# cipherflow-fhe/lattisense

Measured on AMD Instinct MI355X. Metric: ckks_hmult_relin_rescale_throughput, higher is better.
Workload: dtype u64

## Files before the change

lattisense_amd/csrc/build_flags.h:

```cpp
#pragma once

#if (defined(LSA_NTT_DIAG_NO_TWIDDLE_LOADS) || defined(LSA_NTT_DIAG_COPY_ONLY) || defined(LSA_NTT_DIAG_COMPUTE_ONLY) || defined(LSA_NTT_DIAG_TW8) || \
     defined(LSA_KS_DIAG_NO_MATH) || defined(LSA_KS_DIAG_NO_STORE) || defined(LSA_BC_DIAG_NO_MATH) || defined(LSA_BC_DIAG_NO_STORE)) && \
    !defined(LSA_DIAG_BUILD)
#error "wrong-result diagnostic switches need -DLSA_DIAG_BUILD (use lattisense_amd.build --variant: it adds the flag and renames the library)"
#endif

#define LSA_BF_STR2(x) #x
#define LSA_BF_STR(x) LSA_BF_STR2(x)

#define LSA_BUILD_FLAGS_TEXT_1 ""
#ifdef LSA_DIAG_BUILD
#define LSA_BF_DIAG " LSA_DIAG_BUILD"
#else
#define LSA_BF_DIAG ""
#endif
#ifdef LSA_NTT_DIAG_NO_TWIDDLE_LOADS
#define LSA_BF_A " LSA_NTT_DIAG_NO_TWIDDLE_LOADS"
#else
#define LSA_BF_A ""
#endif
#ifdef LSA_NTT_DIAG_COPY_ONLY
#define LSA_BF_B " LSA_NTT_DIAG_COPY_ONLY"
#else
// ... 89 lines not shown
#else
#define LSA_BF_T ""
#endif
#if defined(LSA_NTT_HEAD_ROUNDS) && LSA_NTT_HEAD_ROUNDS != 2
#define LSA_BF_U " LSA_NTT_HEAD_ROUNDS=" LSA_BF_STR(LSA_NTT_HEAD_ROUNDS)
#else
#define LSA_BF_U ""
#endif
#ifdef LSA_R16_BARRIERS
#define LSA_BF_X " LSA_R16_BARRIERS"
#else
#define LSA_BF_X ""
#endif
#if defined(LSA_R16_WAVES) && LSA_R16_WAVES != 4
#define LSA_BF_Y " LSA_R16_WAVES=" LSA_BF_STR(LSA_R16_WAVES)
#else
#define LSA_BF_Y ""
#endif
#ifdef LSA_NTT_NO_LAZY
#define LSA_BF_Z " LSA_NTT_NO_LAZY"
#else
#define LSA_BF_Z ""
#endif
#ifdef LSA_SHOUP_SINGLE_ASM
#define LSA_BF_AA " LSA_SHOUP_SINGLE_ASM"
#else
#define LSA_BF_AA ""
#endif
#ifdef LSA_AB_DPP_LO
#define LSA_BF_AB " LSA_AB_DPP_LO"
#else
#define LSA_BF_AB ""
#endif
#if defined(LSA_KSMAC_WAVES) && LSA_KSMAC_WAVES != 2
#define LSA_BF_AC " LSA_KSMAC_WAVES=" LSA_BF_STR(LSA_KSMAC_WAVES)
#else
#define LSA_BF_AC ""
#endif
#if defined(LSA_KSMAC_WAVES_FP) && LSA_KSMAC_WAVES_FP != 2
#define LSA_BF_AE " LSA_KSMAC_WAVES_FP=" LSA_BF_STR(LSA_KSMAC_WAVES_FP)
#else
#define LSA_BF_AE ""
#endif
#if defined(LSA_KSMAC_CHUNK) && LSA_KSMAC_CHUNK != 4
#define LSA_BF_AF " LSA_KSMAC_CHUNK=" LSA_BF_STR(LSA_KSMAC_CHUNK)
#else
#define LSA_BF_AF ""
#endif
#if defined(LSA_KSMAC_TWCACHE) && LSA_KSMAC_TWCACHE != 1
#define LSA_BF_AH " LSA_KSMAC_TWCACHE=" LSA_BF_STR(LSA_KSMAC_TWCACHE)
#else
#define LSA_BF_AH ""
#endif
#ifdef LSA_NTT_DIAG_TW8
#define LSA_BF_AD " LSA_NTT_DIAG_TW8"
#else
#define LSA_BF_AD ""
#endif
#ifdef LSA_LIFT_ROW_OUTER
#define LSA_BF_AG " LSA_LIFT_ROW_OUTER"
#else
#define LSA_BF_AG ""
#endif
#ifdef LSA_VARIANT_NAME
#define LSA_BF_V " variant=" LSA_BF_STR(LSA_VARIANT_NAME)
#else
#define LSA_BF_V ""
#endif
#ifdef LSA_AB_SWITCH
#define LSA_BF_W " LSA_AB_SWITCH=" LSA_BF_STR(LSA_AB_SWITCH)
#else
#define LSA_BF_W ""
#endif

#define LSA_BUILD_FLAGS_TEXT                                                                                              \
    LSA_BF_DIAG LSA_BF_A LSA_BF_B LSA_BF_C LSA_BF_D LSA_BF_E LSA_BF_F LSA_BF_G LSA_BF_H LSA_BF_I LSA_BF_J LSA_BF_K LSA_BF_L \
        LSA_BF_M LSA_BF_N LSA_BF_O LSA_BF_P LSA_BF_Q LSA_BF_R LSA_BF_S LSA_BF_T LSA_BF_U LSA_BF_V LSA_BF_W LSA_BF_X LSA_BF_Y LSA_BF_Z LSA_BF_AA LSA_BF_AB LSA_BF_AC LSA_BF_AD LSA_BF_AE LSA_BF_AF LSA_BF_AG LSA_BF_AH
```

lattisense_amd/csrc/emu_ntt.cpp:

```cpp
#define LSA_EMULATE 1
#include <cstddef>
#include <vector>
#include "ntt_plan.h"
#include "ntt_chunk.h"
#include "ntt_r16.h"
#include <array>
#include "tables.h"

template <int NT>
static void emu_block(const NttPassArgs& a, const NttBlockCtx& bc, u64* lds) {
    for (int t = 0; t < NT; t++) ntt_phase_load<true, NT, true>(a, bc, t, lds);
    int rho[4];
    const int np = ntt_split(a.mu, rho);
    if (!a.inverse) {
        int sig = 0;
        for (int i = 0; i < np; i++) {
            for (int t = 0; t < NT; t++) ntt_phase_sub_dyn<NT>(a, bc, t, lds, sig, rho[i]);
            sig += rho[i];
        }
    } else {
        int sig = a.mu;
        for (int i = np - 1; i >= 0; i--) {
            sig -= rho[i];
            for (int t = 0; t < NT; t++) ntt_phase_sub_dyn<NT>(a, bc, t, lds, sig, rho[i]);
        }
    }
    for (int t = 0; t < NT; t++) ntt_phase_store<true, NT>(a, bc, t, lds);
}

template <int PASS, int MU, int FZ = 3 | 16>
static void emu_block_r16(const NttPassArgs& a, const NttBlockCtx& bc, u64* lds) {
    std::vector<std::array<u64, 16>> regs(LSA_R16_THREADS);
    for (int phase = 0; phase < 3; phase++)
        for (int t = 0; t < LSA_R16_THREADS; t++) {
            u64(&v)[16] = *reinterpret_cast<u64(*)[16]>(regs[t].data());
            r16_phase<PASS, FZ, MU>(a, bc, t, lds, phase, v);
        }
}

static void emu_block_r8x3(const NttPassArgs& a, const NttBlockCtx& bc, u64* lds) {
    std::vector<std::array<u64, 16>> regs(LSA_R16_THREADS);
    for (int phase = 0; phase < 4; phase++)
        for (int t = 0; t < LSA_R16_THREADS; t++) {
            u64(&v)[16] = *reinterpret_cast<u64(*)[16]>(regs[t].data());
            r8x3_phase<3 | 16>(a, bc, t, lds, phase, v);
        }
}

static int emu_ntt(int n, const u64* moduli, int nmod, u64* data, int batch, long long batch_stride, int rows,
                   const unsigned char* mod_of, int period, int inverse, int tau_max, int allow_fp64, const u64* pa, const u64* pb,
                   const u64* lift = nullptr, int lift_mod = 0, int lift_limbs = 1, int chunk = 0, long long sa = -1,
                   long long sb = -1, long long slift = -1) {
    const int row_inner = (allow_fp64 >> 1) & 1;
    const bool r16 = (allow_fp64 >> 2) & 1;
    allow_fp64 &= 1;
    lsa::HostTables T;
    T.build(n, std::vector<u64>(moduli, moduli + nmod));
    NttPlan plan = make_ntt_plan(T.logn, tau_max);
    std::vector<u64> tw_i(T.psi.size());
    std::vector<double> tw_d(T.psi_d.size());
    for (int m = 0; m < nmod; m++) {
        const size_t o = (size_t)m * n;
        ntt_permute_twiddles(plan, T.logn, (inverse ? T.psiinv : T.psi).data() + 2 * o, tw_i.data() + 2 * o, 2, false);
        ntt_permute_twiddles(plan, T.logn, (inverse ? T.psiinv_d : T.psi_d).data() + o, tw_d.data() + o, 1, true);
    }
    NttPassArgs a{};
    a.src = data;
    a.dst = data;
    a.src_stride = batch_stride;
    a.dst_stride = batch_stride;
    a.batch = batch;
    a.rows = rows;
    a.mods = T.mods.data();
    a.tw = tw_i.data();
    a.scale = T.scale.data();
    a.twd = tw_d.data();
    a.scaled = T.scale_d.data();
    a.allow_fp64 = allow_fp64;
    a.period = period;
    a.row0 = 0;
    a.row_step = 1;
    a.row_inner = row_inner;
    for (int i = 0; i < period; i++) a.mod_of[i] = mod_of[i];
    if (pa) {
        a.fz_pro = 3;
        a.fz_limbs = rows;
        a.fz_a = pa;
        a.fz_b = pb;
        a.fz_a_stride = sa >= 0 ? sa : batch_stride;
        a.fz_b_stride = sb >= 0 ? sb : batch_stride;
        a.fz_a_rpp = a.fz_b_rpp = rows;
    }
    if (lift) {
        a.fz_pro = 4;
        a.fz_limbs = lift_limbs;
        a.fz_last = lift;
        a.fz_last_stride = slift >= 0 ? slift : (long long)(rows / lift_limbs) * n;
        a.fz_last_rpp = 1;
        a.fz_ql_mod = lift_mod;
    }
    int launch_rows = 0;
    for (int r = 0; r < rows; r++)
        if (mod_of[r % period] != LSA_ROW_SKIP) a.row_tbl[launch_rows++] = (unsigned short)r;
    a.compact = 1;
    a.rows = launch_rows;
    const NttPassArgs whole = a;
    const int items = chunk > 0 && chunk < batch ? chunk : batch;
    for (int b0 = 0; b0 < batch; b0 += items) {
        const int nb = batch - b0 < items ? batch - b0 : items;
        a = ntt_chunk_rebase(whole, b0);
        a.batch = nb;
        a.src = a.dst = data + (long long)b0 * batch_stride;
        for (int step = 0; step < plan.npass; step++) {
            int k = inverse ? plan.npass - 1 - step : step;
            ntt_fill_pass(a, plan, T.logn, k, inverse);
            a.fz_first = step == 0;
            a.fp_raw_out = plan.npass == 2 && step == 0;
            a.fp_raw_in = plan.npass == 2 && step == 1;
            std::vector<u64> lds(lds_words(a.tau));
            long long nblocks = (long long)nb * launch_rows * (1 << (a.logn - a.tau));
            for (long long bid = 0; bid < nblocks; bid++) {
                NttBlockCtx bc = ntt_decode_block(a, bid);
                if (bc.mod == LSA_ROW_SKIP) continue;
                if (r16 && ntt_r16_shape_ok(a, plan.npass)) {
                    if (a.mu == 9) emu_block_r8x3(a, bc, lds.data());
                    else if (a.lambda && lift) (a.mu == 8 ? emu_block_r16<0, 8, 32> : emu_block_r16<0, 7, 32>)(a, bc, lds.data());
                    else if (a.lambda && a.mu == 8) emu_block_r16<0, 8>(a, bc, lds.data());
                    else if (a.lambda) emu_block_r16<0, 7>(a, bc, lds.data());
                    else if (a.mu == 8) emu_block_r16<1, 8>(a, bc, lds.data());
                    else emu_block_r16<1, 7>(a, bc, lds.data());
                } else if (a.tau <= 12) emu_block<LSA_NTT_THREADS>(a, bc, lds.data());
                else if (a.tau == 13) emu_block<512>(a, bc, lds.data());
                else emu_block<1024>(a, bc, lds.data());
            }
        }
    }
    return 0;
}

extern "C" int lsa_emu_ntt(int n, const u64* moduli, int nmod, u64* data, int batch, long long batch_stride, int rows,
                           const unsigned char* mod_of, int period, int inverse, int tau_max, int allow_fp64) {
    return emu_ntt(n, moduli, nmod, data, batch, batch_stride, rows, mod_of, period, inverse, tau_max, allow_fp64, nullptr, nullptr);
}

extern "C" int lsa_emu_intt_prod(int n, const u64* moduli, int nmod, const u64* pa, const u64* pb, u64* out, int batch,
                                 long long batch_stride, int rows, const unsigned char* mod_of, int period, int tau_max,
                                 int allow_fp64) {
    if (!pa || !pb) return -1;
    return emu_ntt(n, moduli, nmod, out, batch, batch_stride, rows, mod_of, period, 1, tau_max, allow_fp64, pa, pb);
}

extern "C" int lsa_emu_ntt_lift(int n, const u64* moduli, int nmod, const u64* src, int src_mod, int limbs, u64* out, int batch,
                                long long batch_stride, int rows, const unsigned char* mod_of, int period, int tau_max,
                                int allow_fp64) {
    if (!src || limbs < 1 || rows % limbs || src_mod < 0 || src_mod + rows / limbs > nmod) return -1;
    return emu_ntt(n, moduli, nmod, out, batch, batch_stride, rows, mod_of, period, 0, tau_max, allow_fp64, nullptr, nullptr, src,
                   src_mod, limbs);
}

extern "C" int lsa_emu_intt_prod_chunked(int n, const u64* moduli, int nmod, const u64* pa, long long sa, const u64* pb, long long sb,
                                         u64* out, int batch, long long batch_stride, int rows, const unsigned char* mod_of,
                                         int period, int tau_max, int allow_fp64, int chunk) {
    if (!pa || !pb || sa < 0 || sb < 0 || chunk < 0) return -1;
    return emu_ntt(n, moduli, nmod, out, batch, batch_stride, rows, mod_of, period, 1, tau_max, allow_fp64, pa, pb, nullptr, 0, 1,
                   chunk, sa, sb);
}

extern "C" int lsa_emu_ntt_lift_chunked(int n, const u64* moduli, int nmod, const u64* src, long long src_stride, int src_mod,
                                        int limbs, u64* out, int batch, long long batch_stride, int rows,
                                        const unsigned char* mod_of, int period, int tau_max, int allow_fp64, int chunk) {
    if (!src || src_stride < 0 || limbs < 1 || rows % limbs || src_mod < 0 || src_mod + rows / limbs > nmod || chunk < 0) return -1;
    return emu_ntt(n, moduli, nmod, out, batch, batch_stride, rows, mod_of, period, 0, tau_max, allow_fp64, nullptr, nullptr, src,
// ... 3 lines not shown
```

lattisense_amd/csrc/kernels.hip:

```cpp
#include <atomic>
#include <cstdlib>

#include "build_flags.h"
#include "ks_mac_groups.h"
#include "lsa_internal.h"
#include "ntt_r16.h"
#include "plain_ops.h"
#include "poly_lincomb.h"
#include "tensor_sum.h"

namespace lsa {

const char* kernels_build_flags() { return LSA_BUILD_FLAGS_TEXT; }

static constexpr int TPB = 256;

#ifndef LSA_NTT_WAVES
#define LSA_NTT_WAVES 4
#endif

#if defined(LSA_NTT_DIAG_STAMPS)
#define LSA_STAMP(k)                                                                               \
    do {                                                                                           \
        if (a.diag && threadIdx.x == 0 && blockIdx.x < 8192) a.diag[blockIdx.x * 8 + (k)] = __builtin_amdgcn_s_memtime(); \
// ... 54 lines not shown
    __syncthreads();
    ntt_butterfly_phases<NT>(a, bc, tid, lds);
    if (lds[lds_addr(tid)] == 0x123456789abcull) a.dst[bc.base_dst + tid] = 1;
    return;
#endif
    LSA_STAMP(0);
    ntt_phase_load<(FZ & 1) != 0, NT, (FZ & 16) != 0>(a, bc, tid, lds);
    if (TWL && tid < (1 << a.mu)) {
        u64* tw_l = lds + lds_words(a.tau);
        if (bc.fp) tw_l[tid] = twp.x;
        else {
            tw_l[2 * tid] = twp.x;
            tw_l[2 * tid + 1] = twp.y;
        }
    }
    LSA_STAMP(1);
    __syncthreads();
    LSA_STAMP(2);
#if defined(LSA_NTT_DIAG_COPY_ONLY)
    ntt_phase_store<(FZ & 2) != 0, NT, (FZ & 4) != 0, (FZ & 8) != 0>(a, bc, tid, lds);
    return;
#endif
    ntt_butterfly_phases<NT, TWL>(a, bc, tid, lds);
    ntt_phase_store<(FZ & 2) != 0, NT, (FZ & 4) != 0, (FZ & 8) != 0>(a, bc, tid, lds);
    LSA_STAMP(7);
}

template <int PASS>
__device__ __forceinline__ void r16_sync() {
#if defined(LSA_R16_BARRIERS)
    __syncthreads();
#else
    if (PASS == 0) {
        __syncthreads();
    } else {
        __builtin_amdgcn_fence(__ATOMIC_RELEASE, "wavefront");
        __builtin_amdgcn_wave_barrier();
        __builtin_amdgcn_fence(__ATOMIC_ACQUIRE, "wavefront");
    }
#endif
}
#ifndef LSA_R16_WAVES
#define LSA_R16_WAVES 4
#endif
template <int PASS, int FZ, int MU>
__global__ __launch_bounds__(LSA_R16_THREADS, (FZ & 1) ? LSA_NTT_WAVES_FUSED : LSA_R16_WAVES) void k_ntt_r16(NttPassArgs a) {
    extern __shared__ __attribute__((aligned(16))) u64 lds[];
    const int tid = threadIdx.x;
    const NttBlockCtx bc = ntt_decode_block(a, (long long)blockIdx.x);
    if (bc.mod == LSA_ROW_SKIP) return;
    u64 v[16];
    r16_phase<PASS, FZ, MU>(a, bc, tid, lds, 0, v);
    if (!(PASS == 0 && a.inverse)) r16_sync<PASS>();
    r16_phase<PASS, FZ, MU>(a, bc, tid, lds, 1, v);
    if (PASS == 0 && !a.inverse) return;
    r16_sync<PASS>();
    r16_phase<PASS, FZ, MU>(a, bc, tid, lds, 2, v);
}
template <int FZ>
__global__ __launch_bounds__(LSA_R16_THREADS, LSA_R16_WAVES) void k_ntt_r8x3(NttPassArgs a) {
    extern __shared__ __attribute__((aligned(16))) u64 lds[];
    const int tid = threadIdx.x;
    const NttBlockCtx bc = ntt_decode_block(a, (long long)blockIdx.x);
    if (bc.mod == LSA_ROW_SKIP) return;
    u64 v[16];
    r8x3_phase<FZ>(a, bc, tid, lds, 0, v);
    r16_sync<1>();
    r8x3_phase<FZ>(a, bc, tid, lds, 1, v);
    r16_sync<1>();
    r8x3_phase<FZ>(a, bc, tid, lds, 2, v);
    r16_sync<1>();
    r8x3_phase<FZ>(a, bc, tid, lds, 3, v);
}
static int ntt_pass_fz(const NttPassArgs& a, bool fused) {
    const bool pro = fused && a.fz_pro && a.fz_first, epi = fused && a.fz_epi && a.final_reduce;
    if (pro && a.fz_pro == 3) return 16;
    if (epi && a.fz_epi == 3) return 4;
    if (epi && a.fz_epi == 4) return 8;
    return (pro ? 1 : 0) | (epi ? 2 : 0);
}
template <int FZ>
static auto ntt_r16_second_pass(int mu) {
    return mu == 9 ? &k_ntt_r8x3<FZ> : mu == 8 ? &k_ntt_r16<1, FZ, 8> : &k_ntt_r16<1, FZ, 7>;
}
static bool ntt_launch_r16(const NttPassArgs& a, int npass, bool fused, long long nblocks, hipStream_t s) {
    if (!sw::ntt_r16() || !ntt_r16_shape_ok(a, npass)) return false;
    const int fz = ntt_pass_fz(a, fused);
    void (*k)(NttPassArgs) = nullptr;
    if (a.lambda) {
        if (fz == 1 && a.fz_pro == 4 && sw::r16_pro()) k = a.mu == 8 ? &k_ntt_r16<0, 32, 8> : &k_ntt_r16<0, 32, 7>;
        else if (fz == 1 && a.fz_pro != 4 && a.mu == 8 && sw::r16_pro()) k = &k_ntt_r16<0, 1, 8>;
        else if (fz == 0) k = a.mu == 8 ? &k_ntt_r16<0, 0, 8> : &k_ntt_r16<0, 0, 7>;
    } else if (a.mu != 9 || sw::ntt_r8x3()) {
        switch (fz) {
            case 0: k = ntt_r16_second_pass<0>(a.mu); break;
            case 2: k = ntt_r16_second_pass<2>(a.mu); break;
            case 4: k = ntt_r16_second_pass<4>(a.mu); break;
            case 8: k = ntt_r16_second_pass<8>(a.mu); break;
            case 16: k = a.inverse ? ntt_r16_second_pass<16>(a.mu) : nullptr; break;
        }
    }
    if (!k) return false;
    hipLaunchKernelGGL(k, dim3((unsigned)nblocks), dim3(LSA_R16_THREADS), (size_t)LSA_R16_LDS_WORDS * sizeof(u64), s, a);
    LSA_HIP(hipGetLastError());
    return true;
}

#ifndef LSA_KSMAC_WAVES
#define LSA_KSMAC_WAVES 2
#endif
#ifndef LSA_KSMAC_WAVES_FP
#define LSA_KSMAC_WAVES_FP LSA_KSMAC_WAVES
#endif
template <int MU, bool FP, bool TAIL = false>
__global__ __launch_bounds__(LSA_R16_THREADS, FP ? LSA_KSMAC_WAVES_FP : LSA_KSMAC_WAVES) void k_ntt_r16_ksmac(KsFusedArgs g) {
    static_assert(!TAIL || (FP && MU <= 8), "the tail runs on the FP64 engine's eight- and seven-stage passes");
    extern __shared__ __attribute__((aligned(16))) u64 lds[];
    const int tid = threadIdx.x;
    const int T = g.L + g.np;
    long long bid = blockIdx.x;
    long long b;
    if (g.xcd_deal) {
        const long long slot = bid >> 3;
        b = slot % g.batch;
        bid = (slot / g.batch) * 8 + (bid & 7);
    } else {
        b = bid % g.batch;
        bid /= g.batch;
    }
    const int tl = g.tl_list[bid % g.n_tl], tile = (int)(bid / g.n_tl);
    NttPassArgs a;
    a.logn = g.logn;
    a.s_lo = g.logn - MU;
    a.mu = MU;
    a.lambda = 0;
    a.tau = 12;
    a.inverse = 0;
    a.apply_scale = 0;
    a.final_reduce = 1;
    a.fp_raw_in = g.fp_raw_in;
    a.fp_raw_out = 0;
    a.mods = g.mods;
    a.tw = g.tw;
    a.twd = g.twd;
    a.scale = nullptr;
    a.scaled = nullptr;
    a.src = g.ext;
    a.fz_pro = a.fz_epi = 0;
    a.fz_first = 0;
    NttBlockCtx bc;
    bc.tile = tile;
    bc.mod = tl < g.L ? tl : g.nq + (tl - g.L);
    bc.fp = FP;
    bc.b = (int)b;
    bc.row = 0;
    bc.tw_l = nullptr;
// ... 2379 lines not shown
```

lattisense_amd/csrc/ntt_core.h:

```cpp
#pragma once
#include "modarith.h"

#ifndef LSA_NTT_THREADS
#define LSA_NTT_THREADS 256
#endif
#define LSA_MAX_PERIOD 192
#if defined(LSA_EMULATE)
#include <cstdio>
#include <cstdlib>
#define LSA_EMU_CHECK(c) do { if (!(c)) { std::fprintf(stderr, "ntt replay: range invariant violated: %s (%s:%d)\n", #c, __FILE__, __LINE__); std::abort(); } } while (0)
#else
#define LSA_EMU_CHECK(c) do { } while (0)
#endif
#define LSA_ROW_SKIP 0xFF
#define LSA_FP64_MAX_BITS 47
#ifndef LSA_NTT_MAX_RHO
#define LSA_NTT_MAX_RHO 4
#endif

struct NttPassArgs {
    const u64* src;
    u64* dst;
    long long src_stride;
    long long dst_stride;
// ... 698 lines not shown
    const u64* pa;
    const u64* pb;
    const int half = 1 << (a.tau - 1);
    const NttStoreFix f = ntt_make_store_fix<FZ>(a, bc, g, pa, pb);
    const NttTileMap tm = ntt_tile_map(a, bc.tile);
    if (half == LSA_NTT_STAGE_PAIRS * NT) {
        for (int p0 = 0; p0 < LSA_NTT_STAGE_PAIRS; p0 += LSA_NTT_STORE_CHUNK) {
            u64 v[2 * LSA_NTT_STORE_CHUNK], va[2 * LSA_NTT_STORE_CHUNK], vb[2 * LSA_NTT_STORE_CHUNK];
            int xs[LSA_NTT_STORE_CHUNK];
#pragma unroll
            for (int p = 0; p < LSA_NTT_STORE_CHUNK; p++) {
                const int l = 2 * (tid + (p0 + p) * NT);
                const int x = ntt_tile_index(tm, l);
                xs[p] = x;
                v[2 * p] = lds[lds_addr(l)];
                v[2 * p + 1] = lds[lds_addr(l + 1)];
                va[2 * p] = va[2 * p + 1] = vb[2 * p] = vb[2 * p + 1] = 0;
                if (f.tail) {
                    ntt_load_data_pair(pa + x, va[2 * p], va[2 * p + 1]);
                }
                if (f.with_base) {
                    ntt_load_data_pair(pb + x, vb[2 * p], vb[2 * p + 1]);
                }
            }
            if (FZ && f.tail && a.fz_scatter) {
#pragma unroll
                for (int p = 0; p < LSA_NTT_STORE_CHUNK; p++) {
                    g[a.fz_scatter[xs[p]]] = ntt_store_fix(f, v[2 * p], va[2 * p], vb[2 * p]);
                    g[a.fz_scatter[xs[p] + 1]] = ntt_store_fix(f, v[2 * p + 1], va[2 * p + 1], vb[2 * p + 1]);
                }
                continue;
            }
#pragma unroll
            for (int p = 0; p < LSA_NTT_STORE_CHUNK; p++)
                ntt_store_pair(g + xs[p], ntt_store_fix(f, v[2 * p], va[2 * p], vb[2 * p]),
                               ntt_store_fix(f, v[2 * p + 1], va[2 * p + 1], vb[2 * p + 1]));
        }
        return;
    }
    for (int i = tid; i < half; i += NT) {
        const int x = ntt_tile_index(tm, 2 * i);
        const u64 a0 = f.tail ? pa[x] : 0, a1 = f.tail ? pa[x + 1] : 0;
        const u64 b0 = f.with_base ? pb[x] : 0, b1 = f.with_base ? pb[x + 1] : 0;
        const u64 w0 = ntt_store_fix(f, lds[lds_addr(2 * i)], a0, b0), w1 = ntt_store_fix(f, lds[lds_addr(2 * i + 1)], a1, b1);
        if (FZ && f.tail && a.fz_scatter) {
            g[a.fz_scatter[x]] = w0;
            g[a.fz_scatter[x + 1]] = w1;
        } else {
            ntt_store_pair(g + x, w0, w1);
        }
    }
}

template <int RHO, bool TWU, bool lazy>
LSA_HD void ntt_group_int_impl(u64 (&v)[1 << RHO], bool inverse, const u64* tw , int s_base, unsigned G, u64 q_,
                               bool scale_here, u64 sc0, u64 sc0s, u64 sc1, u64 sc1s) {
    constexpr int E = 1 << RHO;
    const u64 q = q_;
#if defined(LSA_NTT_EXACT_BFLY)
    const u64 q2 = 2 * q;
#else
    const u64 q4 = 4 * q, nq = 0 - q, nq4 = 0 - q4;
#endif
    if (!inverse) {
#pragma unroll
        for (int j = 0; j < RHO; j++) {
            const int half = E >> (j + 1);
            const int s = s_base + j;
            const u64* tws = tw + 2 * (1LL << s);
            u64 w[E / 2], ws[E / 2];
#if defined(LSA_NTT_DIAG_TW8)
            if (!TWU) {
                double wd[E / 2];
                ntt_load_tw_fp(reinterpret_cast<const double*>(tw) + (1LL << s), s, j, G, wd);
#pragma unroll
                for (int k = 0; k < (1 << j); k++) {
                    w[k] = (u64)__builtin_bit_cast(long long, wd[k]);
                    ws[k] = (w[k] << 3) | 1;
                }
            } else
#endif
#pragma unroll
            for (int k = 0; k < (1 << j); k++) {
                if (TWU) {
                    w[k] = LSA_CONST_PTR(u64, tws)[2 * ntt_tw_u_int(s, j, k) + 2u * ntt_tw_v_int(j, G)];
                    ws[k] = LSA_CONST_PTR(u64, tws)[2 * ntt_tw_u_int(s, j, k) + 2u * ntt_tw_v_int(j, G) + 1];
                } else {
                    ntt_load_pair(tws + 2 * ntt_tw_u_int(s, j, k) + 2u * ntt_tw_v_int(j, G), w[k], ws[k]);
                }
            }
#pragma unroll
            for (int e = 0; e < E; e++) {
                if ((e & half) == 0) {
                    const int k = e >> (RHO - j);
#if defined(LSA_NTT_DIAG_NO_TWIDDLE_LOADS)
                    const u64 wk = (u64)(G + 2 * k + 3), wsk = (u64)(G + 2 * k + 5) << 40;
#else
                    const u64 wk = w[k], wsk = ws[k];
#endif
#if defined(LSA_NTT_EXACT_BFLY)
                    u64 U = csub(v[e], q2);
                    u64 T = shoup_mul_lazy(v[e + half], wk, wsk, q);
                    v[e] = U + T;
                    v[e + half] = sub64(U + q2, T);
#else
                    u64 T = shoup_mul_approx(v[e + half], wk, wsk, nq);
                    u64 U;
                    if (lazy) {
                        U = v[e];
                        LSA_EMU_CHECK(U < 0 - 2 * q4 && T < q4);
                    } else {
                        U = csub_sign(v[e], nq4);
                        LSA_EMU_CHECK(v[e] < 2 * q4 && U < q4 && T < q4);
                    }
                    v[e] = U + T;
                    v[e + half] = sub64(U + q4, T);
#endif
                }
            }
        }
    } else {
#pragma unroll
        for (int j = RHO - 1; j >= 0; j--) {
            const int half = E >> (j + 1);
            const int s = s_base + j;
            if (j == 0 && scale_here) {
#pragma unroll
                for (int e = 0; e < half; e++) {
                    u64 U = v[e], V = v[e + half];
                    v[e] = shoup_mul_lazy(U + V, sc0, sc0s, q);
#if defined(LSA_NTT_EXACT_BFLY)
                    v[e + half] = shoup_mul_lazy(sub64(U + q2, V), sc1, sc1s, q);
#else
                    v[e + half] = shoup_mul_lazy(sub64(U + q4, V), sc1, sc1s, q);
#endif
                }
                continue;
            }
            const u64* tws = tw + 2 * (1LL << s);
            u64 w[E / 2], ws[E / 2];
#if defined(LSA_NTT_DIAG_TW8)
            if (!TWU) {
                double wd[E / 2];
                ntt_load_tw_fp(reinterpret_cast<const double*>(tw) + (1LL << s), s, j, G, wd);
#pragma unroll
                for (int k = 0; k < (1 << j); k++) {
                    w[k] = (u64)__builtin_bit_cast(long long, wd[k]);
                    ws[k] = (w[k] << 3) | 1;
                }
            } else
#endif
#pragma unroll
            for (int k = 0; k < (1 << j); k++) {
                if (TWU) {
                    w[k] = LSA_CONST_PTR(u64, tws)[2 * ntt_tw_u_int(s, j, k) + 2u * ntt_tw_v_int(j, G)];
                    ws[k] = LSA_CONST_PTR(u64, tws)[2 * ntt_tw_u_int(s, j, k) + 2u * ntt_tw_v_int(j, G) + 1];
                } else {
                    ntt_load_pair(tws + 2 * ntt_tw_u_int(s, j, k) + 2u * ntt_tw_v_int(j, G), w[k], ws[k]);
                }
            }
#pragma unroll
            for (int e = 0; e < E; e++) {
                if ((e & half) == 0) {
                    const int k = e >> (RHO - j);
                    u64 U = v[e], V = v[e + half];
#if defined(LSA_NTT_DIAG_NO_TWIDDLE_LOADS)
                    const u64 wk = (u64)(G + 2 * k + 3), wsk = (u64)(G + 2 * k + 5) << 40;
#else
                    const u64 wk = w[k], wsk = ws[k];
#endif
#if defined(LSA_NTT_EXACT_BFLY)
                    v[e] = csub(U + V, q2);
                    v[e + half] = shoup_mul_lazy(sub64(U + q2, V), wk, wsk, q);
#else
                    LSA_EMU_CHECK(U < q4 && V < q4);
                    v[e] = csub_sign(U + V, nq4);
                    v[e + half] = shoup_mul_approx(sub64(U + q4, V), wk, wsk, nq);
                    LSA_EMU_CHECK(v[e] < q4 && v[e + half] < q4);
#endif
                }
            }
        }
    }
}

template <int RHO, bool TWU = false>
LSA_HD void ntt_group_int(u64 (&v)[1 << RHO], bool inverse, const u64* tw, int s_base, unsigned G, u64 q, bool scale_here, u64 sc0, u64 sc0s,
                          u64 sc1, u64 sc1s) {
    if (!inverse && ntt_int_lazy(q)) ntt_group_int_impl<RHO, TWU, true>(v, false, tw, s_base, G, q, false, 0, 0, 0, 0);
    else ntt_group_int_impl<RHO, TWU, false>(v, inverse, tw, s_base, G, q, scale_here, sc0, sc0s, sc1, sc1s);
}

template <int RHO, bool LIN, int NT, bool TWL = false>
LSA_HD void ntt_phase_sub(const NttPassArgs& a, const NttBlockCtx& bc, int tid, u64* lds, int sig0) {
    constexpr int E = 1 << RHO;
    const ModDev md = a.mods[bc.mod];
    const u64* tw = TWL ? bc.tw_l : a.tw + (((long long)bc.mod << a.logn) << 1);
    const int beta0 = a.lambda + a.mu - sig0 - RHO;
    const int ngroups = 1 << (a.tau - RHO);
    const bool scale_here = a.inverse && a.apply_scale && a.s_lo + sig0 == 0;
    const u64* sc = a.scale + 4 * bc.mod;
    const u64 sc0 = scale_here ? sc[0] : 0, sc0s = scale_here ? sc[1] : 0, sc1 = scale_here ? sc[2] : 0, sc1s = scale_here ? sc[3] : 0;
    for (int gid = tid; gid < ngroups; gid += NT) {
        int lbase = ((gid >> beta0) << (beta0 + RHO)) | (gid & ((1 << beta0) - 1));
        const int ad0 = lds_addr(lbase), adst = !LIN ? 0 : beta0 ? (1 << beta0) + (1 << (beta0 - 4)) : 1;
        u64 v[E];
#pragma unroll
        for (int e = 0; e < E; e++) v[e] = lds[LIN ? ad0 + e * adst : lds_addr(lbase + (e << beta0))];
        int r = (lbase >> a.lambda) & ((1 << a.mu) - 1);
        int H = ntt_hi_index(a, bc.tile, lbase);
        int G = (H << sig0) + (r >> (a.mu - sig0));
        ntt_group_int<RHO>(v, a.inverse != 0, tw, a.s_lo + sig0, (unsigned)G, md.q, scale_here, sc0, sc0s, sc1, sc1s);
#pragma unroll
        for (int e = 0; e < E; e++) lds[LIN ? ad0 + e * adst : lds_addr(lbase + (e << beta0))] = v[e];
    }
}

template <int RHO, bool TWU = false, bool TWC = false>
LSA_HD void ntt_group_fp(double (&v)[1 << RHO], bool inverse, const double* tw , int s_base, unsigned G, double q, double qinv,
                         bool scale_here, double sc0, double sc1, bool long_pass, const double* twc = nullptr) {
    constexpr int E = 1 << RHO;
    if (!inverse) {
#pragma unroll
        for (int j = 0; j < RHO; j++) {
            const int half = E >> (j + 1);
            const int s = s_base + j;
            double w[E / 2];
            if (TWC) {
#pragma unroll
                for (int k = 0; k < (1 << j); k++) w[k] = twc[(1 << j) - 1 + k];
            } else if (TWU) {
#pragma unroll
                for (int k = 0; k < (1 << j); k++) w[k] = LSA_CONST_PTR(double, tw + (1LL << s))[ntt_tw_pos_fp(s, j, G, k)];
            } else {
                ntt_load_tw_fp(tw + (1LL << s), s, j, G, w);
            }
#pragma unroll
            for (int e = 0; e < E; e++) {
                if ((e & half) == 0) {
#if defined(LSA_NTT_DIAG_NO_TWIDDLE_LOADS)
                    const double T = fp_modmul(v[e + half], (double)(G + j + 3), q, qinv);
#else
                    const double T = fp_modmul(v[e + half], w[e >> (RHO - j)], q, qinv);
#endif
                    const double U = v[e];
                    LSA_EMU_CHECK(__builtin_fabs(U) < 2251799813685248.0 && __builtin_fabs(v[e + half]) < 2251799813685248.0);
                    v[e] = U + T;
                    v[e + half] = U - T;
                }
            }
        }
        if (long_pass) {
#pragma unroll
            for (int e = 0; e < E; e++) v[e] = fp_reduce(v[e], q, qinv);
        }
    } else {
#pragma unroll
        for (int j = RHO - 1; j >= 0; j--) {
            const int half = E >> (j + 1);
            const int s = s_base + j;
            if (j == 0 && scale_here) {
#pragma unroll
                for (int e = 0; e < half; e++) {
                    const double U = v[e], V = v[e + half];
                    v[e] = fp_modmul(U + V, sc0, q, qinv);
                    v[e + half] = fp_modmul(U - V, sc1, q, qinv);
                }
                continue;
            }
            double w[E / 2];
            if (TWC) {
#pragma unroll
                for (int k = 0; k < (1 << j); k++) w[k] = twc[(1 << j) - 1 + k];
            } else if (TWU) {
#pragma unroll
                for (int k = 0; k < (1 << j); k++) w[k] = LSA_CONST_PTR(double, tw + (1LL << s))[ntt_tw_pos_fp(s, j, G, k)];
            } else {
                ntt_load_tw_fp(tw + (1LL << s), s, j, G, w);
            }
#pragma unroll
            for (int e = 0; e < E; e++) {
                if ((e & half) == 0) {
                    const double U = v[e], V = v[e + half];
                    v[e] = U + V;
                    v[e + half] = fp_modmul(U - V, w[e >> (RHO - j)], q, qinv);
                }
            }
        }
#pragma unroll
        for (int e = 0; e < E; e++) v[e] = fp_reduce(v[e], q, qinv);
    }
}

template <int RHO, bool LIN, int NT, bool TWL = false>
LSA_HD void ntt_phase_sub_fp(const NttPassArgs& a, const NttBlockCtx& bc, int tid, u64* lds, int sig0) {
    constexpr int E = 1 << RHO;
    const double q = (double)a.mods[bc.mod].q, qinv = 1.0 / q;
    const double* tw = TWL ? reinterpret_cast<const double*>(bc.tw_l) : a.twd + ((long long)bc.mod << a.logn);
    const int beta0 = a.lambda + a.mu - sig0 - RHO;
    const int ngroups = 1 << (a.tau - RHO);
    const bool scale_here = a.inverse && a.apply_scale && a.s_lo + sig0 == 0;
    const double sc0 = scale_here ? a.scaled[2 * bc.mod] : 0.0, sc1 = scale_here ? a.scaled[2 * bc.mod + 1] : 0.0;
    for (int gid = tid; gid < ngroups; gid += NT) {
        int lbase = ((gid >> beta0) << (beta0 + RHO)) | (gid & ((1 << beta0) - 1));
        const int ad0 = lds_addr(lbase), adst = !LIN ? 0 : beta0 ? (1 << beta0) + (1 << (beta0 - 4)) : 1;
        double v[E];
#pragma unroll
        for (int e = 0; e < E; e++) v[e] = d_from_bits(lds[LIN ? ad0 + e * adst : lds_addr(lbase + (e << beta0))]);
        int r = (lbase >> a.lambda) & ((1 << a.mu) - 1);
        int H = ntt_hi_index(a, bc.tile, lbase);
        int G = (H << sig0) + (r >> (a.mu - sig0));
        ntt_group_fp<RHO>(v, a.inverse != 0, tw, a.s_lo + sig0, (unsigned)G, q, qinv, scale_here, sc0, sc1, a.mu > 9);
#pragma unroll
        for (int e = 0; e < E; e++) lds[LIN ? ad0 + e * adst : lds_addr(lbase + (e << beta0))] = d_to_bits(v[e]);
    }
}

LSA_HD int ntt_split(int mu, int* rho ) {
    const int n = (mu + LSA_NTT_MAX_RHO - 1) / LSA_NTT_MAX_RHO;
    if ((mu > 12 || mu == 10) && LSA_NTT_MAX_RHO == 4) {
        for (int i = 0; i < n; i++) rho[i] = 4;
        rho[n - 2] = mu - 4 * (n - 1);
        return n;
    }
// ... 45 lines not shown
```

lattisense_amd/csrc/ntt_r16.h:

```cpp
#pragma once
#include "ntt_core.h"

#define LSA_R16_THREADS 256
#define LSA_R16_LDS_WORDS (272 * 16)

LSA_HD bool ntt_r16_shape_ok(const NttPassArgs& a, int npass) {
    if (npass != 2 || a.tau != 12) return false;
    if (a.mu == 9) return a.s_lo == a.logn - 9 && a.lambda == 0;
    if (a.mu != 8 && a.mu != 7) return false;
    return (a.s_lo == 0 && a.lambda == 12 - a.mu) || (a.s_lo == a.logn - a.mu && a.lambda == 0);
}

template <int PASS, int MU>
LSA_HD int r16_lds(int k, int i) {
    const int p = i + (i >> 4);
    return PASS == 0 ? (p << (12 - MU)) + k : k * ((1 << MU) + (1 << (MU - 4))) + p;
}
template <int PASS, int MU>
LSA_HD long long r16_x(const NttPassArgs& a, int tile, int k, int i) {
    return PASS == 0 ? ((long long)tile << (12 - MU)) + ((long long)i << (a.logn - MU)) + k : ((long long)tile << 12) + (k << MU) + i;
}
template <int MU, int IMAGE>
LSA_HD int r16_pt(int i, int e) {
    return IMAGE == 0 ? i + (e << (MU - 4)) : 16 * i + e;
// ... 337 lines not shown
            for (int j = 0; j < 2 * LSA_NTT_STORE_CHUNK; j++) {
                double r = f.skip_reduce ? d_from_bits(v[j]) : fp_reduce(d_from_bits(v[j]), f.qd, f.qinvd);
                if (r < 0) r += f.qd;
                w[j] = double_to_u52(r);
            }
        } else {
#pragma unroll
            for (int j = 0; j < 2 * LSA_NTT_STORE_CHUNK; j++) w[j] = ntt_store_fix(f, v[j], va[j], vb[j]);
        }
        if (FZ && f.tail && a.fz_scatter) {
#pragma unroll
            for (int m = 0; m < LSA_NTT_STORE_CHUNK; m++) {
                g[a.fz_scatter[xs[m]]] = w[2 * m];
                g[a.fz_scatter[xs[m] + 1]] = w[2 * m + 1];
            }
            continue;
        }
#pragma unroll
        for (int m = 0; m < LSA_NTT_STORE_CHUNK; m++) ntt_store_pair(g + xs[m], w[2 * m], w[2 * m + 1]);
    }
}

#if defined(LSA_AB_DPP_LO) && defined(__HIP_DEVICE_COMPILE__)
template <int D>
__device__ __forceinline__ int r16_dpp_xor32(int v) {
    if (D == 8) return __builtin_amdgcn_update_dpp(0, v, 0x128, 0xF, 0xF, false);
    if (D == 2) return __builtin_amdgcn_update_dpp(0, v, 0x4E, 0xF, 0xF, false);
    if (D == 1) return __builtin_amdgcn_update_dpp(0, v, 0xB1, 0xF, 0xF, false);
    int r = __builtin_amdgcn_update_dpp(0, v, 0x124, 0xF, 0xA, false);
    return __builtin_amdgcn_update_dpp(r, v, 0x12C, 0xF, 0x5, false);
}
template <int D>
__device__ __forceinline__ double r16_dpp_xor(double x) {
    const u64 b = d_to_bits(x);
    const u32 lo = (u32)r16_dpp_xor32<D>((int)(u32)b), hi = (u32)r16_dpp_xor32<D>((int)(u32)(b >> 32));
    return d_from_bits(((u64)hi << 32) | lo);
}
template <int J>
__device__ __forceinline__ void r16_dpp_stage(double (&v)[16], const double* twd, int s_lo, unsigned G1, int i_hi, double q, double qinv) {
    constexpr int D = 8 >> J;
    const int s = s_lo + J, kk = i_hi >> (4 - J);
    const double w = (twd + (1LL << s))[ntt_tw_pos_fp(s, J, G1, kk)];
    const bool upper = (i_hi >> (3 - J)) & 1;
#pragma unroll
    for (int e = 0; e < 16; e++) {
        const double X = v[e], P = r16_dpp_xor<D>(X);
        const double U = upper ? P : X, V = upper ? X : P;
        const double T = fp_modmul(V, w, q, qinv);
        v[e] = upper ? U - T : U + T;
    }
}
#endif

template <int PASS, int FZ, int MU>
LSA_HD void r16_phase(const NttPassArgs& a, const NttBlockCtx& bc, int tid, u64* lds, int phase, u64 (&v)[16]) {
    const R16Limb L = r16_limb(a, bc);
    int k, i;
    r16_lane<PASS, MU>(tid, k, i);
    const unsigned G1 = r16_G1<PASS, MU>(bc, k), G2 = (G1 << 4) + ((unsigned)i << (8 - MU));
#if defined(LSA_AB_DPP_LO) && defined(__HIP_DEVICE_COMPILE__)
    if (PASS == 1 && MU == 8 && !a.inverse && bc.fp) {
        if (phase == 0) {
            r16_load_coalesced<false, MU>(a, bc, tid, lds);
        } else if (phase == 1) {
            r16_lds_get<PASS, 1, MU>(tid, lds, v);
            double d[16];
#pragma unroll
            for (int e = 0; e < 16; e++) d[e] = d_from_bits(v[e]);
            r16_dpp_stage<0>(d, L.twd, L.s_lo, G1, i, L.q, L.qinv);
            r16_dpp_stage<1>(d, L.twd, L.s_lo, G1, i, L.q, L.qinv);
            r16_dpp_stage<2>(d, L.twd, L.s_lo, G1, i, L.q, L.qinv);
            r16_dpp_stage<3>(d, L.twd, L.s_lo, G1, i, L.q, L.qinv);
#pragma unroll
            for (int e = 0; e < 16; e++) v[e] = d_to_bits(d[e]);
            r16_group<PASS, 1, MU>(v, a, bc, L, G2);
            r16_lds_put<PASS, 1, MU>(tid, lds, v);
        } else {
            r16_store_coalesced<(FZ & 2) != 0, MU, (FZ & 4) != 0, (FZ & 8) != 0>(a, bc, tid, lds);
        }
        return;
    }
#endif
    if (!a.inverse) {
        if (phase == 0) {
            r16_load_direct<PASS, (FZ & (1 | 32)) != 0, 0, MU, (FZ & 32) ? 2 : 0>(a, bc, tid, v);
            r16_group<PASS, 0, MU>(v, a, bc, L, G1);
            r16_lds_put<PASS, 0, MU>(tid, lds, v);
        } else if (phase == 1) {
            r16_lds_get<PASS, 1, MU>(tid, lds, v);
            r16_group<PASS, 1, MU>(v, a, bc, L, G2);
            if (PASS == 0) r16_store_direct<PASS, (FZ & 2) != 0, 1, MU>(a, bc, tid, v);
            else r16_lds_put<PASS, 1, MU>(tid, lds, v);
        } else if (PASS == 1) {
            r16_store_coalesced<(FZ & 2) != 0, MU, (FZ & 4) != 0, (FZ & 8) != 0>(a, bc, tid, lds);
        }
    } else {
        if (phase == 0) {
            if (PASS == 0) r16_load_direct<PASS, false, 1, MU>(a, bc, tid, v);
            else r16_load_coalesced<false, MU, (FZ & 16) != 0>(a, bc, tid, lds);
        } else if (phase == 1) {
            if (PASS == 1) r16_lds_get<PASS, 1, MU>(tid, lds, v);
            r16_group<PASS, 1, MU>(v, a, bc, L, G2);
            r16_lds_put<PASS, 1, MU>(tid, lds, v);
        } else {
            r16_lds_get<PASS, 0, MU>(tid, lds, v);
            r16_group<PASS, 0, MU>(v, a, bc, L, G1);
            r16_store_direct<PASS, false, 0, MU>(a, bc, tid, v);
        }
    }
}

template <int IMAGE>
LSA_HD int r8x3_pt(int i, int E) {
    if (IMAGE == 0) return i + (E << 5);
    if (IMAGE == 2) return 16 * i + E;
    return ((2 * (i >> 3) + (E >> 3)) << 6) | ((E & 7) << 3) | (i & 7);
}
template <int IMAGE>
LSA_HD constexpr int r8x3_slot(int g, int e) {
    return IMAGE == 0 ? g + 2 * e : 8 * g + e;
}
template <int IMAGE>
LSA_HD void r8x3_group(u64 (&v)[16], const NttPassArgs& a, const NttBlockCtx& bc, const R16Limb& L, unsigned G1, int i) {
    const int s_base = L.s_lo + 3 * IMAGE;
#pragma unroll
    for (int g = 0; g < 2; g++) {
        const unsigned G = IMAGE == 0 ? G1 : IMAGE == 1 ? (G1 << 3) + 2u * (unsigned)(i >> 3) + (unsigned)g : (G1 << 6) + 2u * (unsigned)i + (unsigned)g;
        if (bc.fp) {
            double d[8];
#pragma unroll
            for (int e = 0; e < 8; e++) d[e] = d_from_bits(v[r8x3_slot<IMAGE>(g, e)]);
            ntt_group_fp<3, false>(d, a.inverse != 0, L.twd, s_base, G, L.q, L.qinv, false, 0.0, 0.0, false);
#pragma unroll
            for (int e = 0; e < 8; e++) v[r8x3_slot<IMAGE>(g, e)] = d_to_bits(d[e]);
        } else {
            u64 w[8];
#pragma unroll
            for (int e = 0; e < 8; e++) w[e] = v[r8x3_slot<IMAGE>(g, e)];
            ntt_group_int<3, false>(w, a.inverse != 0, L.tw, s_base, G, L.md.q, false, 0, 0, 0, 0);
#pragma unroll
            for (int e = 0; e < 8; e++) v[r8x3_slot<IMAGE>(g, e)] = w[e];
        }
    }
}
template <int IMAGE>
LSA_HD void r8x3_put(int k, int i, u64* lds, const u64 (&v)[16]) {
#pragma unroll
    for (int E = 0; E < 16; E++) lds[r16_lds<1, 9>(k, r8x3_pt<IMAGE>(i, E))] = v[E];
}
template <int IMAGE>
LSA_HD void r8x3_get(int k, int i, const u64* lds, u64 (&v)[16]) {
#pragma unroll
    for (int E = 0; E < 16; E++) v[E] = lds[r16_lds<1, 9>(k, r8x3_pt<IMAGE>(i, E))];
}
template <int FZ>
LSA_HD void r8x3_phase(const NttPassArgs& a, const NttBlockCtx& bc, int tid, u64* lds, int phase, u64 (&v)[16]) {
    const R16Limb L = r16_limb(a, bc);
    const int k = tid >> 5, i = tid & 31;
    const unsigned G1 = r16_G1<1, 9>(bc, k);
// ... 310 lines not shown
```

Measured before the change: 16450.

## Share radix-16 NTT twiddles across lanes through an LDS strip

In the eight-stage radix-16 NTT passes, each group of 16 lanes now has its 15 twiddles loaded cooperatively, one per lane, and written to a small per-wave LDS strip. Every lane then reads its stage twiddles from that strip with vector loads instead of issuing its own global twiddle loads. The aim is to cut redundant global and cache traffic for twiddle factors. In exchange the kernel uses extra LDS per workgroup, which is capped so four workgroups still fit per CU, and adds wave-level ordering fences plus an extra barrier in one inverse path.

```diff
diff --git a/lattisense_amd/csrc/build_flags.h b/lattisense_amd/csrc/build_flags.h
--- a/lattisense_amd/csrc/build_flags.h
+++ b/lattisense_amd/csrc/build_flags.h
@@ -165,6 +165,11 @@
 #else
 #define LSA_BF_AH ""
 #endif
+#if defined(LSA_R16_TWSHARE) && LSA_R16_TWSHARE != 1
+#define LSA_BF_AI " LSA_R16_TWSHARE=" LSA_BF_STR(LSA_R16_TWSHARE)
+#else
+#define LSA_BF_AI ""
+#endif
 #ifdef LSA_NTT_DIAG_TW8
 #define LSA_BF_AD " LSA_NTT_DIAG_TW8"
 #else
@@ -188,4 +193,4 @@
 
 #define LSA_BUILD_FLAGS_TEXT                                                                                              \
     LSA_BF_DIAG LSA_BF_A LSA_BF_B LSA_BF_C LSA_BF_D LSA_BF_E LSA_BF_F LSA_BF_G LSA_BF_H LSA_BF_I LSA_BF_J LSA_BF_K LSA_BF_L \
-        LSA_BF_M LSA_BF_N LSA_BF_O LSA_BF_P LSA_BF_Q LSA_BF_R LSA_BF_S LSA_BF_T LSA_BF_U LSA_BF_V LSA_BF_W LSA_BF_X LSA_BF_Y LSA_BF_Z LSA_BF_AA LSA_BF_AB LSA_BF_AC LSA_BF_AD LSA_BF_AE LSA_BF_AF LSA_BF_AG LSA_BF_AH
+        LSA_BF_M LSA_BF_N LSA_BF_O LSA_BF_P LSA_BF_Q LSA_BF_R LSA_BF_S LSA_BF_T LSA_BF_U LSA_BF_V LSA_BF_W LSA_BF_X LSA_BF_Y LSA_BF_Z LSA_BF_AA LSA_BF_AB LSA_BF_AC LSA_BF_AD LSA_BF_AE LSA_BF_AF LSA_BF_AG LSA_BF_AH LSA_BF_AI
diff --git a/lattisense_amd/csrc/emu_ntt.cpp b/lattisense_amd/csrc/emu_ntt.cpp
--- a/lattisense_amd/csrc/emu_ntt.cpp
+++ b/lattisense_amd/csrc/emu_ntt.cpp
@@ -31,11 +31,15 @@
 template <int PASS, int MU, int FZ = 3 | 16>
 static void emu_block_r16(const NttPassArgs& a, const NttBlockCtx& bc, u64* lds) {
     std::vector<std::array<u64, 16>> regs(LSA_R16_THREADS);
-    for (int phase = 0; phase < 3; phase++)
+    constexpr bool TWS = r16_twshare(PASS, 0, MU);
+    for (int phase = 0; phase < 3; phase++) {
+        if (TWS && r16_tws_fill_in_read_phase<PASS>(a.inverse != 0, phase))
+            for (int t = 0; t < LSA_R16_THREADS; t++) r16_tws_fill<PASS>(a, bc, t, lds);
         for (int t = 0; t < LSA_R16_THREADS; t++) {
             u64(&v)[16] = *reinterpret_cast<u64(*)[16]>(regs[t].data());
-            r16_phase<PASS, FZ, MU>(a, bc, t, lds, phase, v);
+            r16_phase<PASS, FZ, MU, TWS>(a, bc, t, lds, phase, v);
         }
+    }
 }
 
 static void emu_block_r8x3(const NttPassArgs& a, const NttBlockCtx& bc, u64* lds) {
@@ -117,7 +121,7 @@
             a.fz_first = step == 0;
             a.fp_raw_out = plan.npass == 2 && step == 0;
             a.fp_raw_in = plan.npass == 2 && step == 1;
-            std::vector<u64> lds(lds_words(a.tau));
+            std::vector<u64> lds(lds_words(a.tau) + R16Tws::WORDS);
             long long nblocks = (long long)nb * launch_rows * (1 << (a.logn - a.tau));
             for (long long bid = 0; bid < nblocks; bid++) {
                 NttBlockCtx bc = ntt_decode_block(a, bid);
diff --git a/lattisense_amd/csrc/kernels.hip b/lattisense_amd/csrc/kernels.hip
--- a/lattisense_amd/csrc/kernels.hip
+++ b/lattisense_amd/csrc/kernels.hip
@@ -130,6 +130,7 @@
     u64 v[16];
     r16_phase<PASS, FZ, MU>(a, bc, tid, lds, 0, v);
     if (!(PASS == 0 && a.inverse)) r16_sync<PASS>();
+    else if (r16_twshare(PASS, FZ, MU)) r16_sync<1>();
     r16_phase<PASS, FZ, MU>(a, bc, tid, lds, 1, v);
     if (PASS == 0 && !a.inverse) return;
     r16_sync<PASS>();
@@ -165,9 +166,12 @@
     if (!sw::ntt_r16() || !ntt_r16_shape_ok(a, npass)) return false;
     const int fz = ntt_pass_fz(a, fused);
     void (*k)(NttPassArgs) = nullptr;
+    int kfz = fz;
     if (a.lambda) {
-        if (fz == 1 && a.fz_pro == 4 && sw::r16_pro()) k = a.mu == 8 ? &k_ntt_r16<0, 32, 8> : &k_ntt_r16<0, 32, 7>;
-        else if (fz == 1 && a.fz_pro != 4 && a.mu == 8 && sw::r16_pro()) k = &k_ntt_r16<0, 1, 8>;
+        if (fz == 1 && a.fz_pro == 4 && sw::r16_pro()) {
+            k = a.mu == 8 ? &k_ntt_r16<0, 32, 8> : &k_ntt_r16<0, 32, 7>;
+            kfz = 32;
+        } else if (fz == 1 && a.fz_pro != 4 && a.mu == 8 && sw::r16_pro()) k = &k_ntt_r16<0, 1, 8>;
         else if (fz == 0) k = a.mu == 8 ? &k_ntt_r16<0, 0, 8> : &k_ntt_r16<0, 0, 7>;
     } else if (a.mu != 9 || sw::ntt_r8x3()) {
         switch (fz) {
@@ -179,7 +183,8 @@
         }
     }
     if (!k) return false;
-    hipLaunchKernelGGL(k, dim3((unsigned)nblocks), dim3(LSA_R16_THREADS), (size_t)LSA_R16_LDS_WORDS * sizeof(u64), s, a);
+    const size_t lds_bytes = r16_plain_lds_bytes(a.mu != 9 && r16_twshare(a.lambda ? 0 : 1, kfz, a.mu));
+    hipLaunchKernelGGL(k, dim3((unsigned)nblocks), dim3(LSA_R16_THREADS), lds_bytes, s, a);
     LSA_HIP(hipGetLastError());
     return true;
 }
diff --git a/lattisense_amd/csrc/ntt_core.h b/lattisense_amd/csrc/ntt_core.h
--- a/lattisense_amd/csrc/ntt_core.h
+++ b/lattisense_amd/csrc/ntt_core.h
@@ -774,9 +774,30 @@
     }
 }
 
-template <int RHO, bool TWU, bool lazy>
+LSA_HD void ntt_twp_stage_int(const u64* twp, int j, u64* w, u64* ws) {
+#pragma unroll
+    for (int k = 0; k < (1 << j); k++) ntt_load_pair(twp + 2 * ((1 << j) - 1 + k), w[k], ws[k]);
+}
+LSA_HD void ntt_twp_stage_fp(const double* twp, int j, double* w) {
+    if (j == 0) {
+        w[0] = twp[0];
+        return;
+    }
+#pragma unroll
+    for (int k = 0; k < (1 << j); k += 2) {
+#if defined(__HIP_DEVICE_COMPILE__)
+        const double2 v = *reinterpret_cast<const double2*>(twp + (1 << j) - 1 + k);
+        w[k] = v.x;
+        w[k + 1] = v.y;
+#else
+        w[k] = twp[(1 << j) - 1 + k];
+        w[k + 1] = twp[(1 << j) + k];
+#endif
+    }
+}
+template <int RHO, bool TWU, bool lazy, bool TWC = false>
 LSA_HD void ntt_group_int_impl(u64 (&v)[1 << RHO], bool inverse, const u64* tw , int s_base, unsigned G, u64 q_,
-                               bool scale_here, u64 sc0, u64 sc0s, u64 sc1, u64 sc1s) {
+                               bool scale_here, u64 sc0, u64 sc0s, u64 sc1, u64 sc1s, const u64* twc = nullptr) {
     constexpr int E = 1 << RHO;
     const u64 q = q_;
 #if defined(LSA_NTT_EXACT_BFLY)
@@ -792,7 +813,7 @@
             const u64* tws = tw + 2 * (1LL << s);
             u64 w[E / 2], ws[E / 2];
 #if defined(LSA_NTT_DIAG_TW8)
-            if (!TWU) {
+            if (!TWU && !TWC) {
                 double wd[E / 2];
                 ntt_load_tw_fp(reinterpret_cast<const double*>(tw) + (1LL << s), s, j, G, wd);
 #pragma unroll
@@ -804,7 +825,9 @@
 #endif
 #pragma unroll
             for (int k = 0; k < (1 << j); k++) {
-                if (TWU) {
+                if (TWC) {
+                    if (k == 0) ntt_twp_stage_int(twc, j, w, ws);
+                } else if (TWU) {
                     w[k] = LSA_CONST_PTR(u64, tws)[2 * ntt_tw_u_int(s, j, k) + 2u * ntt_tw_v_int(j, G)];
                     ws[k] = LSA_CONST_PTR(u64, tws)[2 * ntt_tw_u_int(s, j, k) + 2u * ntt_tw_v_int(j, G) + 1];
                 } else {
@@ -862,7 +885,7 @@
             const u64* tws = tw + 2 * (1LL << s);
             u64 w[E / 2], ws[E / 2];
 #if defined(LSA_NTT_DIAG_TW8)
-            if (!TWU) {
+            if (!TWU && !TWC) {
                 double wd[E / 2];
                 ntt_load_tw_fp(reinterpret_cast<const double*>(tw) + (1LL << s), s, j, G, wd);
 #pragma unroll
@@ -874,7 +897,9 @@
 #endif
 #pragma unroll
             for (int k = 0; k < (1 << j); k++) {
-                if (TWU) {
+                if (TWC) {
+                    if (k == 0) ntt_twp_stage_int(twc, j, w, ws);
+                } else if (TWU) {
                     w[k] = LSA_CONST_PTR(u64, tws)[2 * ntt_tw_u_int(s, j, k) + 2u * ntt_tw_v_int(j, G)];
                     ws[k] = LSA_CONST_PTR(u64, tws)[2 * ntt_tw_u_int(s, j, k) + 2u * ntt_tw_v_int(j, G) + 1];
                 } else {
@@ -906,11 +931,11 @@
     }
 }
 
-template <int RHO, bool TWU = false>
+template <int RHO, bool TWU = false, bool TWC = false>
 LSA_HD void ntt_group_int(u64 (&v)[1 << RHO], bool inverse, const u64* tw, int s_base, unsigned G, u64 q, bool scale_here, u64 sc0, u64 sc0s,
-                          u64 sc1, u64 sc1s) {
-    if (!inverse && ntt_int_lazy(q)) ntt_group_int_impl<RHO, TWU, true>(v, false, tw, s_base, G, q, false, 0, 0, 0, 0);
-    else ntt_group_int_impl<RHO, TWU, false>(v, inverse, tw, s_base, G, q, scale_here, sc0, sc0s, sc1, sc1s);
+                          u64 sc1, u64 sc1s, const u64* twc = nullptr) {
+    if (!inverse && ntt_int_lazy(q)) ntt_group_int_impl<RHO, TWU, true, TWC>(v, false, tw, s_base, G, q, false, 0, 0, 0, 0, twc);
+    else ntt_group_int_impl<RHO, TWU, false, TWC>(v, inverse, tw, s_base, G, q, scale_here, sc0, sc0s, sc1, sc1s, twc);
 }
 
 template <int RHO, bool LIN, int NT, bool TWL = false>
@@ -938,7 +963,7 @@
     }
 }
 
-template <int RHO, bool TWU = false, bool TWC = false>
+template <int RHO, bool TWU = false, bool TWC = false, bool TWP = false>
 LSA_HD void ntt_group_fp(double (&v)[1 << RHO], bool inverse, const double* tw , int s_base, unsigned G, double q, double qinv,
                          bool scale_here, double sc0, double sc1, bool long_pass, const double* twc = nullptr) {
     constexpr int E = 1 << RHO;
@@ -948,7 +973,9 @@
             const int half = E >> (j + 1);
             const int s = s_base + j;
             double w[E / 2];
-            if (TWC) {
+            if (TWC && TWP) {
+                ntt_twp_stage_fp(twc, j, w);
+            } else if (TWC) {
 #pragma unroll
                 for (int k = 0; k < (1 << j); k++) w[k] = twc[(1 << j) - 1 + k];
             } else if (TWU) {
@@ -991,7 +1018,9 @@
                 continue;
             }
             double w[E / 2];
-            if (TWC) {
+            if (TWC && TWP) {
+                ntt_twp_stage_fp(twc, j, w);
+            } else if (TWC) {
 #pragma unroll
                 for (int k = 0; k < (1 << j); k++) w[k] = twc[(1 << j) - 1 + k];
             } else if (TWU) {
diff --git a/lattisense_amd/csrc/ntt_r16.h b/lattisense_amd/csrc/ntt_r16.h
--- a/lattisense_amd/csrc/ntt_r16.h
+++ b/lattisense_amd/csrc/ntt_r16.h
@@ -413,8 +413,102 @@
 }
 #endif
 
-template <int PASS, int FZ, int MU>
+#ifndef LSA_R16_TWSHARE
+#define LSA_R16_TWSHARE 1
+#endif
+struct R16Tws {
+    static constexpr int WAVE = 2 * 17 * 4;
+    static constexpr int WORDS = (LSA_R16_THREADS / 64) * WAVE;
+    static LSA_HD int fp(int tid, int e) { return (tid >> 6) * WAVE + 18 * ((tid >> 4) & 3) + 1 + e; }
+    static LSA_HD int pair(int tid, int e) { return (tid >> 6) * WAVE + 2 * (17 * ((tid >> 4) & 3) + e); }
+};
+constexpr bool r16_twshare(int pass, int fz, int mu) { return LSA_R16_TWSHARE != 0 && mu == 8 && (fz == 0 || fz == 2); }
+constexpr size_t r16_plain_lds_bytes(bool tws) { return (size_t)(LSA_R16_LDS_WORDS + (tws ? R16Tws::WORDS : 0)) * sizeof(u64); }
+static_assert(r16_plain_lds_bytes(true) <= 40960, "four workgroups per CU");
+LSA_HD int r16_tws_entry(int tid) { return (tid & 15) - 1; }
+template <int PASS>
+LSA_HD bool r16_tws_fill_in_read_phase(bool inverse, int phase) {
+    return PASS == 1 && !inverse && phase == 0;
+}
+LSA_HD void r16_wave_order() {
+#if defined(__HIP_DEVICE_COMPILE__)
+    __builtin_amdgcn_fence(__ATOMIC_RELEASE, "wavefront");
+    __builtin_amdgcn_wave_barrier();
+    __builtin_amdgcn_fence(__ATOMIC_ACQUIRE, "wavefront");
+#endif
+}
+struct R16TwsVal {
+    u64 x, y;
+};
+template <int PASS>
+LSA_HD R16TwsVal r16_tws_load(const R16Limb& L, bool fp, int tid, unsigned G) {
+    R16TwsVal t = {0, 0};
+    const int e = r16_tws_entry(tid);
+    if (e < 0) return t;
+    const int j = 31 - __builtin_clz((unsigned)(e + 1)), k = e + 1 - (1 << j), s = (PASS == 0 ? 4 : L.s_lo) + j;
+    if (fp) t.x = d_to_bits((L.twd + (1LL << s))[ntt_tw_pos_fp(s, j, G, k)]);
+    else ntt_load_pair(L.tw + 2 * (1LL << s) + 2 * ntt_tw_pos_int(s, j, G, k), t.x, t.y);
+    return t;
+}
+LSA_HD void r16_tws_store(u64* strip, bool fp, int tid, const R16TwsVal& t) {
+    const int e = r16_tws_entry(tid);
+    if (e < 0) return;
+    if (fp) {
+        strip[R16Tws::fp(tid, e)] = t.x;
+        return;
+    }
+    u64* p = strip + R16Tws::pair(tid, e);
+#if defined(__HIP_DEVICE_COMPILE__)
+    *reinterpret_cast<ulonglong2*>(p) = make_ulonglong2(t.x, t.y);
+#else
+    p[0] = t.x;
+    p[1] = t.y;
+#endif
+}
+template <int PASS>
+LSA_HD unsigned r16_tws_G(const NttBlockCtx& bc, int tid) {
+    int k, i;
+    r16_lane<PASS, 8>(tid, k, i);
+    return PASS == 0 ? (unsigned)i : r16_G1<PASS, 8>(bc, k);
+}
+template <int PASS>
+LSA_HD void r16_tws_fill(const NttPassArgs& a, const NttBlockCtx& bc, int tid, u64* lds) {
+    r16_tws_store(lds + LSA_R16_LDS_WORDS, bc.fp != 0, tid, r16_tws_load<PASS>(r16_limb(a, bc), bc.fp != 0, tid, r16_tws_G<PASS>(bc, tid)));
+}
+LSA_HD const double* r16_tws_slot_fp(const u64* strip, int tid) { return reinterpret_cast<const double*>(strip) + R16Tws::fp(tid, 0); }
+LSA_HD const u64* r16_tws_slot_int(const u64* strip, int tid) { return strip + R16Tws::pair(tid, 0); }
+LSA_HD void r16_tws_get_fp(const u64* strip, int tid, double (&w)[15]) {
+#pragma unroll
+    for (int j = 0; j < 4; j++) ntt_twp_stage_fp(r16_tws_slot_fp(strip, tid), j, w + (1 << j) - 1);
+}
+LSA_HD void r16_tws_get_int(const u64* strip, int tid, u64 (&w)[30]) {
+    u64 x[8], y[8];
+#pragma unroll
+    for (int j = 0; j < 4; j++) {
+        ntt_twp_stage_int(r16_tws_slot_int(strip, tid), j, x, y);
+#pragma unroll
+        for (int k = 0; k < (1 << j); k++) {
+            w[2 * ((1 << j) - 1 + k)] = x[k];
+            w[2 * ((1 << j) - 1 + k) + 1] = y[k];
+        }
+    }
+}
+LSA_HD void r16_group_tws(u64 (&v)[16], bool inverse, bool fp, const R16Limb& L, const u64* strip, int tid) {
+    if (fp) {
+        double d[16];
+#pragma unroll
+        for (int e = 0; e < 16; e++) d[e] = d_from_bits(v[e]);
+        ntt_group_fp<4, false, true, true>(d, inverse, nullptr, 0, 0u, L.q, L.qinv, false, 0.0, 0.0, false, r16_tws_slot_fp(strip, tid));
+#pragma unroll
+        for (int e = 0; e < 16; e++) v[e] = d_to_bits(d[e]);
+    } else {
+        ntt_group_int<4, false, true>(v, inverse, nullptr, 0, 0u, L.md.q, false, 0, 0, 0, 0, r16_tws_slot_int(strip, tid));
+    }
+}
+
+template <int PASS, int FZ, int MU, bool TWS = r16_twshare(PASS, FZ, MU)>
 LSA_HD void r16_phase(const NttPassArgs& a, const NttBlockCtx& bc, int tid, u64* lds, int phase, u64 (&v)[16]) {
+    static_assert(!TWS || MU == 8, "the strip's layout is the eight-stage passes'");
     const R16Limb L = r16_limb(a, bc);
     int k, i;
     r16_lane<PASS, MU>(tid, k, i);
@@ -442,14 +536,27 @@
         return;
     }
 #endif
+    const bool fp = bc.fp != 0, inv = a.inverse != 0;
+    u64* const strip = lds + LSA_R16_LDS_WORDS;
+    const unsigned GS = PASS == 0 ? G2 : G1;
+    if (TWS && phase == 0 && PASS == 0) r16_tws_store(strip, fp, tid, r16_tws_load<PASS>(L, fp, tid, GS));
     if (!a.inverse) {
         if (phase == 0) {
+            R16TwsVal tv = {0, 0};
+            if (TWS && PASS == 1) tv = r16_tws_load<PASS>(L, fp, tid, GS);
             r16_load_direct<PASS, (FZ & (1 | 32)) != 0, 0, MU, (FZ & 32) ? 2 : 0>(a, bc, tid, v);
-            r16_group<PASS, 0, MU>(v, a, bc, L, G1);
+            if (TWS && PASS == 1) {
+                r16_tws_store(strip, fp, tid, tv);
+                r16_wave_order();
+                r16_group_tws(v, inv, fp, L, strip, tid);
+            } else {
+                r16_group<PASS, 0, MU>(v, a, bc, L, G1);
+            }
             r16_lds_put<PASS, 0, MU>(tid, lds, v);
         } else if (phase == 1) {
             r16_lds_get<PASS, 1, MU>(tid, lds, v);
-            r16_group<PASS, 1, MU>(v, a, bc, L, G2);
+            if (TWS && PASS == 0) r16_group_tws(v, inv, fp, L, strip, tid);
+            else r16_group<PASS, 1, MU>(v, a, bc, L, G2);
             if (PASS == 0) r16_store_direct<PASS, (FZ & 2) != 0, 1, MU>(a, bc, tid, v);
             else r16_lds_put<PASS, 1, MU>(tid, lds, v);
         } else if (PASS == 1) {
@@ -457,15 +564,18 @@
         }
     } else {
         if (phase == 0) {
+            if (TWS && PASS == 1) r16_tws_store(strip, fp, tid, r16_tws_load<PASS>(L, fp, tid, GS));
             if (PASS == 0) r16_load_direct<PASS, false, 1, MU>(a, bc, tid, v);
             else r16_load_coalesced<false, MU, (FZ & 16) != 0>(a, bc, tid, lds);
         } else if (phase == 1) {
             if (PASS == 1) r16_lds_get<PASS, 1, MU>(tid, lds, v);
-            r16_group<PASS, 1, MU>(v, a, bc, L, G2);
+            if (TWS && PASS == 0) r16_group_tws(v, inv, fp, L, strip, tid);
+            else r16_group<PASS, 1, MU>(v, a, bc, L, G2);
             r16_lds_put<PASS, 1, MU>(tid, lds, v);
         } else {
             r16_lds_get<PASS, 0, MU>(tid, lds, v);
-            r16_group<PASS, 0, MU>(v, a, bc, L, G1);
+            if (TWS && PASS == 1) r16_group_tws(v, inv, fp, L, strip, tid);
+            else r16_group<PASS, 0, MU>(v, a, bc, L, G1);
             r16_store_direct<PASS, false, 0, MU>(a, bc, tid, v);
         }
     }
```

Result: no change. 16600, median of 6 (+0.9%).
